# kennege/pvnet

Hardware: AMD Instinct MI355X
Metric: images/sec (480x640, 9 kp) vote->keypoint (higher is better)
Workload: dtype f32; 1 GPU; stream of LINEMOD-cat-sized batch-1 frames (configs[1]'s voting layer): ransac_voting_layer_v3 (hn=512, thr=0.99) from seg_pred/vertex_pred; one step = one hipGraph replay voting 1024 frames per GPU, 8 in flight on separate streams; images sharded round-robin over ranks, one gather of all keypoints at the end; global_batch=1024, keypoints=9, round_hyp_num=512, foreground_px=29861, parallelism=dp1 (images sharded round-robin, RCCL all_gather of keypoints), images_in_flight=8, stream_images=169984

## Files before the change

### pvnet_amd/csrc/pvvote.hip

```cpp
#include "pv_stages.h"

#define PV_VERSION "pvvote 0.2 (gfx950)"

#ifdef PVV_TRACE
#define PVV_TRACE_ON(a) ((a).trace != nullptr)
#else
#define PVV_TRACE_ON(a) false
#endif

#ifdef PVV_PROFILE
namespace pvv __attribute__((visibility("hidden"))) {
int g_abl = 0;
}
#endif

namespace {

using namespace pvv;

struct alignas(16) F4 { float x, y, z, w; };
struct alignas(8) F2 { float x, y; };

struct VoteArgs {
    const float4 *pex;
// ... 541 lines not shown
#endif

__global__ __launch_bounds__(256) void k_hyp_gen(VoteArgs a) {
    const int64_t per = (int64_t)a.nh * a.vn;
    const int64_t gid = (int64_t)blockIdx.x * 256 + threadIdx.x;
    if (gid >= per * a.b) return;
    const int b = (int)(gid / per);
    const int r = (int)(gid - b * per);
    const int h = r / a.vn, v = r - h * a.vn;
    const int n = tn_at(a, b);
    if (n > 0) a.hypv_out[((int64_t)b * a.vn + v) * a.nh + h] = item_hyp<true, true>(a, b, v, h, true, n, true);
}

typedef _Float16 h4f __attribute__((ext_vector_type(4)));
typedef float f32x16 __attribute__((ext_vector_type(16)));

constexpr int kMB = 16;
constexpr int kMChunk = PVM_CHUNK;
constexpr int kMSlots = (kMChunk + 255) / 256;
constexpr int kMBatch = kMChunk / kMB;
static_assert(kMChunk % kMB == 0 && kMBatch <= 32 && kMChunk <= 512, "hit masks: 2 x 64 bits; queue: 9-bit pixel");
constexpr int kMSet = 4;
constexpr float kMHypMax = 8.0e6f;
constexpr float kMRMax = 30000.f;
constexpr int kMQueue = PVM_QUEUE;
constexpr int kMBandK = 1;

template <bool PREPPED>
struct MSlab {
    uint4 rows[kMBatch][2 * kMB];
    ExactSlab<PREPPED, kMChunk> x;
};

__device__ __forceinline__ uint32_t pack_h2(_Float16 lo, _Float16 hi) {
    return (uint32_t)__builtin_bit_cast(uint16_t, lo) | ((uint32_t)__builtin_bit_cast(uint16_t, hi) << 16);
}

__device__ __forceinline__ uint4 form_row(float ax, float ay, float b) {
    const _Float16 axh = (_Float16)ax, axl = (_Float16)(ax - (float)axh);
    const _Float16 ayh = (_Float16)ay, ayl = (_Float16)(ay - (float)ayh);
    const float nb = -b;
    const _Float16 bh = (_Float16)nb, bl = (_Float16)(nb - (float)bh);
    return make_uint4(pack_h2(axh, axh), pack_h2(axl, ayh), pack_h2(ayh, ayl), pack_h2(bh, bl));
}

template <bool PREPPED>
__global__ __launch_bounds__(256) __attribute__((amdgpu_waves_per_eu(PVM_WPE, PVM_WPE))) void k_vote_mfma(VoteArgs a) {
    const int lane = lane_id();
    const int wid = (int)__builtin_amdgcn_readfirstlane(threadIdx.x / kWave);
    const int col = lane & 31, half = lane >> 5;
    const int unit = (int)blockIdx.x;
    const uint32_t nunits = gridDim.x;
    const uint64_t t_start = __builtin_amdgcn_s_memrealtime();
    __builtin_amdgcn_s_setprio(3);
    __shared__ MSlab<PREPPED> slab[2];
    __shared__ QuarterBoxes qb_all[2];
    __shared__ float2 hyp_all[4 * kGroup];
    __shared__ uint32_t bq_all[4][kMQueue];
    __shared__ int32_t corr_all[4][kGroup];
    float2 *hlds = hyp_all + wid * kGroup;
    uint32_t *bq = bq_all[wid];
    int32_t *corr = corr_all[wid];
    const int ggn = a.hgn / 4;
    uint32_t total = 0;
    for (int b = 0; b < a.b; ++b) total += (uint32_t)(a.vn * ggn) * (uint32_t)tn_at(a, b);
    uint32_t lo, hi;
    if (a.rw[0] > 0 && nunits % (a.rw[3] > 0 ? 4 : 3) == 0) {
        round_share(total, nunits, (uint32_t)unit, a.rw, &lo, &hi);
    } else {
        even_share(total, nunits, (uint32_t)unit, &lo, &hi);
    }
    int buf = 0, nfix = 0, nseg = 0, nslow = 0, nxo = 0, nqd = 0;
    uint64_t tloop = 0, t_total = 0, t_hyp = 0;
    uint64_t c_stage = 0, c_hot = 0, c_fix = 0, c_seg = 0, c_mark = 0;
    uint64_t c_band = 0, c_flush = 0, c_xo = 0;
    auto cyc = [&]() -> uint64_t { return PVV_TRACE_ON(a) ? __builtin_amdgcn_s_memtime() : 0; };
    if (PVV_TRACE_ON(a)) t_total = __builtin_amdgcn_s_memrealtime();
    const float tau = a.tau;
    constexpr float kBig = 3.0e38f;
    int b = 0;
    uint32_t base = 0;
    while (lo < hi && b < a.b) {
        const int n = tn_at(a, b);
        const uint32_t span = (uint32_t)(a.vn * ggn) * (uint32_t)n;
        if (lo >= base + span) { base += span; ++b; continue; }
        const uint32_t r0 = lo - base;
        const int g = (int)(r0 / (uint32_t)n);
        const int ts = uniform((int)(r0 - (uint32_t)g * n));
        const int te = uniform((int)min((uint32_t)n, ts + (hi - lo)));
        const int v = uniform(g / ggn), gg = g - (g / ggn) * ggn;
        const int hg = uniform(gg * 4 + wid);
        c_mark = cyc();
        F4 L[kMSlots];
        auto load_px = [&](int s0, int np) {
#pragma unroll
            for (int k = 0; k < kMSlots; ++k) {
                const int t = k * 256 + wid * kWave + lane;
                L[k] = F4{0.f, 0.f, 0.f, 0.f};
                if (t < np) L[k] = pixel_exact<PREPPED>(a, b, v, s0 + t);
            }
        };
        load_px(ts, min(kMChunk, te - ts));
        uint32_t hfm = 0, hxm = 0;
#pragma unroll
        for (int i = 0; i < 2; ++i) {
            const int h = hg * kGroup + i * kWave + lane;
            const bool hl = h < a.nh;
            const float2 hv = a.hyp ? item_hyp<false, PREPPED>(a, b, v, h, hl, n, false)
                                    : item_hyp<PREPPED, PREPPED>(a, b, v, h, hl, n, PREPPED && ts == 0);
            hlds[i * kWave + lane] = hv;
        }
        __builtin_amdgcn_wave_barrier();
#pragma unroll
        for (int j = 0; j < kMSet; ++j) {
            const int h = hg * kGroup + j * 32 + col;
            const float2 hv = hlds[j * 32 + col];
            const bool fin = isfinite(hv.x) && isfinite(hv.y);
            const bool xo = h < a.nh && fin &&
                            (hyp_exact_only(hv.x, hv.y) || !(fabsf(hv.x) < kMHypMax && fabsf(hv.y) < kMHypMax));
            hxm |= xo ? 1u << j : 0u;
            hfm |= (h < a.nh && fin && !xo) ? 1u << j : 0u;
        }
        int cnt[kMSet] = {0, 0, 0, 0};
        corr[lane] = 0;
        corr[64 + lane] = 0;
        if (PVV_TRACE_ON(a) && t_hyp == 0) t_hyp = __builtin_amdgcn_s_memrealtime();
        for (int s0 = ts; s0 < te; s0 += kMChunk) {
            {
                const uint64_t t = cyc();
                if (s0 == ts) c_seg += t - c_mark; else c_fix += t - c_mark;
                c_mark = t;
            }
            const int np = uniform(min(kMChunk, te - s0));
            MSlab<PREPPED> &S = slab[buf];
            QuarterBoxes &QB = qb_all[buf];
            buf ^= 1;
            const int t = wid * kWave + lane;
            bool exo_p = false;
            float xl = kBig, xh = -kBig;
            float4 q[kMSlots];
            float yq[kMSlots];
#pragma unroll
            for (int k = 0; k < kMSlots; ++k) {
                const int tt = k * 256 + t;
                q[k] = make_float4(__builtin_nanf(""), 0.f, 0.f, 0.f);
                yq[k] = 0.f;
                if (tt < np) {
                    const F4 e = L[k];
                    bool ex = false;
                    if (PREPPED) q[k] = prep_compacted(e, &ex);
                    else { q[k] = prep_pixel(e.x, e.y, e.z, e.w); ex = pixel_exotic(e.z, e.w); }
                    exo_p |= ex;
                    S.x.put(tt, e);
                    xl = fminf(xl, e.x); xh = fmaxf(xh, e.x); yq[k] = q[k].y;
                }
            }
            if (wid * kWave < np) {
                const float mn = wave_min(xl), mx = wave_max(xh);
                float yn, yx;
                if (PREPPED) {
                    yn = bcast(yq[0], 0);
                    const bool s1 = kMSlots > 1 && 256 + wid * kWave < np;
                    yx = s1 ? bcast(yq[kMSlots - 1], min(kWave - 1, np - 1 - 256 - wid * kWave))
                            : bcast(yq[0], min(kWave - 1, np - 1 - wid * kWave));
                } else {
                    float mnq = kBig, mxq = -kBig;
#pragma unroll
                    for (int k = 0; k < kMSlots; ++k)
                        if (k * 256 + t < np) { mnq = fminf(mnq, yq[k]); mxq = fmaxf(mxq, yq[k]); }
                    yn = wave_min(mnq);
                    yx = wave_max(mxq);
                }
                const uint32_t ex = __builtin_amdgcn_ballot_w64(exo_p) != 0;
                if (lane == 0) { QB.box[wid] = make_float4(mn, mx, yn, yx); QB.exo[wid] = ex; }
            } else if (lane == 0) {
                QB.box[wid] = make_float4(kBig, -kBig, kBig, -kBig);
                QB.exo[wid] = 0;
            }
            auto put_rows = [&](float ox, float oy, bool slow) {
#pragma unroll
                for (int k = 0; k < kMSlots; ++k) {
                    const int tt = k * 256 + t;
                    if (tt >= kMChunk) break;
                    uint4 rx = make_uint4(0u, 0u, pack_h2((_Float16)0.f, (_Float16)0.f),
                                          pack_h2((_Float16)(-60000.f), (_Float16)0.f));
                    uint4 ry = make_uint4(0u, 0u, 0u, 0u);
                    if (q[k].x == q[k].x && !slow) {
                        const float cx = q[k].x - ox, cy = q[k].y - oy;
                        const float axX = tau * q[k].z, ayX = tau * q[k].w;
                        rx = form_row(axX, ayX, fmaf(axX, cx, ayX * cy));
                        ry = form_row(-q[k].w, q[k].z, fmaf(-q[k].w, cx, q[k].z * cy));
                    }
                    S.rows[tt >> 4][2 * (tt & 15)] = rx;
                    S.rows[tt >> 4][2 * (tt & 15) + 1] = ry;
                }
            };
            if (s0 + kMChunk < te) load_px(s0 + kMChunk, min(kMChunk, te - s0 - kMChunk));
            __syncthreads();
            float cxl = kBig, cxh = -kBig, cyl = kBig, cyh = -kBig;
            uint32_t exq = 0;
#pragma unroll
            for (int k = 0; k < 4; ++k) {
                const float4 Q = QB.box[k];
                cxl = fminf(cxl, Q.x); cxh = fmaxf(cxh, Q.y);
                cyl = fminf(cyl, Q.z); cyh = fmaxf(cyh, Q.w);
                exq |= QB.exo[k];
            }
            float ox = floorf(0.5f * cxl + 0.5f * cxh), oy = floorf(0.5f * cyl + 0.5f * cyh);
            if (!(fabsf(ox) <= 1.6e7f && fabsf(oy) <= 1.6e7f)) { ox = 0.f; oy = 0.f; }
            const float axr = fmaxf(cxh - ox, ox - cxl), ayr = fmaxf(cyh - oy, oy - cyl);
            const float R = __builtin_amdgcn_sqrtf(fmaf(axr, axr, ayr * ayr)) * 1.00001f;
            bool slow = !a.fast || exq != 0 || !(R * fmaxf(tau, 1.f) <= kMRMax);
            slow = __builtin_amdgcn_readfirstlane(slow);
            nslow += slow ? 1 : 0;
            put_rows(ox, oy, slow);
            __syncthreads();
            if (!slow) {
                auto hscale = [&](int j, float &hx, float &hy, float &s, float &Bv) {
                    const bool fj = (hfm >> j) & 1u;
                    const float2 hv = hlds[j * 32 + col];
                    hx = hv.x - ox;
                    hy = hv.y - oy;
                    const float mag = fmaxf(fabsf(hx), fabsf(hy));
                    const int e = __builtin_amdgcn_frexp_expf(mag);
                    const int k = fj ? max(0, e - 14) : 0;
                    s = __builtin_ldexpf(1.f, -k);
                    Bv = (__builtin_amdgcn_sqrtf(fmaf(hx, hx, hy * hy)) * 1.00001f + R) * 1.00001f + 1.f;
                };
                h4f bf[kMSet];
                float gb[kMSet];
#pragma unroll
                for (int j = 0; j < kMSet; ++j) {
                    const bool fj = (hfm >> j) & 1u;
                    float hx, hy, s, Bv;
                    hscale(j, hx, hy, s, Bv);
                    const float hxs = hx * s, hys = hy * s;
                    const _Float16 xh_ = (_Float16)hxs, xl_ = (_Float16)(hxs - (float)xh_);
                    const _Float16 yh_ = (_Float16)hys, yl_ = (_Float16)(hys - (float)yh_);
                    const _Float16 sh = (_Float16)s;
                    h4f f = half ? h4f{yl_, yh_, sh, sh} : h4f{xh_, xl_, xh_, yh_};
                    if (!fj) f = h4f{(_Float16)0.f, (_Float16)0.f, (_Float16)0.f, (_Float16)0.f};
                    bf[j] = f;
                    gb[j] = fj ? (a.gzf + a.gzr) * Bv * s * 1.00001f : -1.f;
                }
                uint32_t neg[kMSet] = {0u, 0u, 0u, 0u};
                uint64_t hm0 = 0, hm1 = 0;
                const int nb = (np + kMB - 1) / kMB;
                const uint2 *arow = (const uint2 *)&S.rows[0][0];
                auto afrag = [&](int p) -> h4f {
                    const uint2 w = arow[(p * kMB * 2 + col) * 2 + half];
                    return __builtin_bit_cast(h4f, w);
                };
                auto zvals = [&](const f32x16 &c, float z[8]) {
#pragma unroll
                    for (int q = 0; q < 8; ++q) z[q] = c[2 * q] - fabsf(c[2 * q + 1]);
                };
                auto proc = [&](const f32x16 &c, uint32_t &ng) -> float {
                    float z[8];
                    zvals(c, z);
#pragma unroll
                    for (int q = 0; q < 8; q += 4) {
                        const uint32_t p01 = __builtin_amdgcn_perm(__float_as_uint(z[q + 1]), __float_as_uint(z[q]), 0x0c0c0b09u);
                        const uint32_t p23 = __builtin_amdgcn_perm(__float_as_uint(z[q + 3]), __float_as_uint(z[q + 2]), 0x0b090c0cu);
                        ng = __builtin_amdgcn_sad_u8(p01, p23, ng);
                    }
                    float mb = __builtin_elementwise_minimum(__builtin_elementwise_minimum(fabsf(z[0]), fabsf(z[1])), fabsf(z[2]));
                    mb = __builtin_elementwise_minimum(__builtin_elementwise_minimum(mb, fabsf(z[3])), fabsf(z[4]));
                    mb = __builtin_elementwise_minimum(__builtin_elementwise_minimum(mb, fabsf(z[5])), fabsf(z[6]));
                    return __builtin_elementwise_minimum(mb, fabsf(z[7]));
                };
                const f32x16 zero = {};
                if (PVV_TRACE_ON(a) && tloop == 0) tloop = __builtin_amdgcn_s_memrealtime();
                { const uint64_t t = cyc(); c_stage += t - c_mark; c_mark = t; }
                h4f A = afrag(0);
                f32x16 c0 = __builtin_amdgcn_mfma_f32_32x32x8f16(A, bf[0], zero, 0, 0, 0);
#pragma unroll 1
                for (int p = 0; p < nb; ++p) {
                    const h4f An = afrag(min(p + 1, kMBatch - 1));
                    const f32x16 c1 = __builtin_amdgcn_mfma_f32_32x32x8f16(A, bf[1], zero, 0, 0, 0);
                    const float m0 = proc(c0, neg[0]);
                    const f32x16 c2 = __builtin_amdgcn_mfma_f32_32x32x8f16(A, bf[2], zero, 0, 0, 0);
                    const float m1 = proc(c1, neg[1]);
                    const f32x16 c3 = __builtin_amdgcn_mfma_f32_32x32x8f16(A, bf[3], zero, 0, 0, 0);
                    const float m2 = proc(c2, neg[2]);
                    c0 = __builtin_amdgcn_mfma_f32_32x32x8f16(An, bf[0], zero, 0, 0, 0);
                    const float m3 = proc(c3, neg[3]);
                    const uint32_t hb = (__builtin_amdgcn_ballot_w64(m0 <= gb[0]) != 0 ? 1u : 0u) |
                                        (__builtin_amdgcn_ballot_w64(m1 <= gb[1]) != 0 ? 2u : 0u) |
                                        (__builtin_amdgcn_ballot_w64(m2 <= gb[2]) != 0 ? 4u : 0u) |
                                        (__builtin_amdgcn_ballot_w64(m3 <= gb[3]) != 0 ? 8u : 0u);
                    const uint64_t hbs = (uint64_t)hb << ((p & 15) * kMSet);
                    if (p < 16) hm0 |= hbs; else hm1 |= hbs;
                    A = An;
                }
#pragma unroll
                for (int j = 0; j < kMSet; ++j) cnt[j] += ((hfm >> j) & 1u) ? 8 * nb - (int)(neg[j] / 255u) : 0;
                { const uint64_t t = cyc(); c_hot += t - c_mark; c_mark = t; }
#ifdef PVV_PROFILE
                if (a.rw[3] == 7777) hm0 = hm1 = 0;
#endif
                const float kx = a.gzr / tau * 1.0001f, ky = a.gzr * 1.0001f;
                int nq = 0;
                auto flush = [&]() {
                    for (int k0 = 0; k0 < nq; k0 += kWave) {
                        if (k0 + lane < nq) {
                            const uint32_t en = bq[k0 + lane];
                            const int pix = (int)(en & 0x1ffu), jj = (int)((en >> 9) & 3u), cl = (int)((en >> 11) & 31u);
                            const int f = (int)(en >> 16) & 1;
                            const F4 e = S.x.get(pix);
                            const float2 hj = hlds[jj * 32 + cl];
                            const int r = exact_vote(e.z, e.w, e.x, e.y, hj.x, hj.y, a.thr) ? 1 : 0;
                            if (r != f) atomicAdd(&corr[jj * 32 + cl], r - f);
                        }
                    }
                    nq = 0;
                };
                const float inv1k = 1.0002f / (1.f - ky * 1.0001f);
                float Gs[kMSet];
                const float gq = a.gzf / (a.gzf + a.gzr) * 1.0011f * inv1k;
#pragma unroll
                for (int j = 0; j < kMSet; ++j) Gs[j] = gb[j] * gq;
                const float Kb = (kx + ky) * inv1k;
                auto band_test = [&](const f32x16 &c, int p, int j) {
                    const bool fj = (hfm >> j) & 1u;
                    const float G = j == 0 ? Gs[0] : j == 1 ? Gs[1] : j == 2 ? Gs[2] : Gs[3];
                    float zs[8], ts[8];
#pragma unroll
                    for (int q = 0; q < 8; ++q) {
                        const float X = c[2 * q], Y = c[2 * q + 1];
                        zs[q] = X - fabsf(Y);
                        ts[q] = fmaf(-Kb, fabsf(X), fabsf(zs[q]));
                    }
                    float mt = __builtin_elementwise_minimum(__builtin_elementwise_minimum(ts[0], ts[1]), ts[2]);
                    mt = __builtin_elementwise_minimum(__builtin_elementwise_minimum(mt, ts[3]), ts[4]);
                    mt = __builtin_elementwise_minimum(__builtin_elementwise_minimum(mt, ts[5]), ts[6]);
                    mt = __builtin_elementwise_minimum(mt, ts[7]);
#ifdef PVV_PROFILE
                    if (a.rw[3] == 7778) mt = 3.0e38f;
#endif
                    if (__builtin_amdgcn_ballot_w64(fj && mt <= G)) {
#pragma unroll
                        for (int q = 0; q < 8; ++q) {
                            const int pix = p * kMB + (q & 1) + 4 * (q >> 1) + 2 * half;
                            const bool u = fj && pix < np && ts[q] <= G;
                            const uint64_t m = __builtin_amdgcn_ballot_w64(u);
                            if (m) {
                                if (nq > kMQueue - kWave) flush();
                                const int at = nq + (int)__builtin_amdgcn_mbcnt_hi((uint32_t)(m >> 32), __builtin_amdgcn_mbcnt_lo((uint32_t)m, 0u));
                                if (u) bq[at] = (uint32_t)pix | ((uint32_t)j << 9) | ((uint32_t)col << 11) | ((signbit(zs[q]) ? 0u : 1u) << 16);
                                nq += __popcll(m);
                                nqd += __popcll(m);
                            }
                        }
                    }
                };
                static_assert(kMSet == 4, "band selects");
                auto bsel = [&](int j) -> h4f { return j == 0 ? bf[0] : j == 1 ? bf[1] : j == 2 ? bf[2] : bf[3]; };
                while (hm0 | hm1) {
                    int pk[kMBandK], jk[kMBandK], nk = 0;
#pragma unroll
                    for (int k = 0; k < kMBandK; ++k) {
                        pk[k] = 0; jk[k] = 0;
                        if (hm0 | hm1) {
                            int bit;
                            if (hm0) { bit = __builtin_ctzll(hm0); hm0 &= hm0 - 1; }
                            else { bit = 64 + __builtin_ctzll(hm1); hm1 &= hm1 - 1; }
                            pk[k] = bit / kMSet; jk[k] = bit % kMSet;
                            nk = k + 1;
                        }
                    }
                    nfix += nk;
                    h4f ak[kMBandK];
#pragma unroll
                    for (int k = 0; k < kMBandK; ++k) ak[k] = afrag(pk[k]);
                    f32x16 ck[kMBandK];
#pragma unroll
                    for (int k = 0; k < kMBandK; ++k)
                        ck[k] = __builtin_amdgcn_mfma_f32_32x32x8f16(ak[k], bsel(jk[k]), zero, 0, 0, 0);
#pragma unroll
                    for (int k = 0; k < kMBandK; ++k)
                        if (k < nk) band_test(ck[k], pk[k], jk[k]);
                }
                { const uint64_t t = cyc(); c_band += t - c_mark; c_fix += t - c_mark; c_mark = t; }
                flush();
                __builtin_amdgcn_wave_barrier();
                { const uint64_t t = cyc(); c_flush += t - c_mark; c_fix += t - c_mark; c_mark = t; }
#pragma unroll
                for (int j = 0; j < kMSet; ++j) {
                    uint64_t mm = __builtin_amdgcn_ballot_w64(((hxm >> j) & 1u) && half == 0);
                    nxo += __popcll(mm);
                    while (mm) {
                        const int l = __builtin_ctzll(mm);
                        mm &= mm - 1;
                        const float2 hx2 = hlds[j * 32 + l];
                        int c = 0;
#pragma unroll
                        for (int k = 0; k < (kMChunk + kWave - 1) / kWave; ++k) {
                            const int jj = k * kWave + lane;
                            bool e = false;
                            if (jj < np) {
                                const F4 x = S.x.get(jj);
                                e = exact_vote(x.z, x.w, x.x, x.y, hx2.x, hx2.y, a.thr);
                            }
                            c += __popcll(__builtin_amdgcn_ballot_w64(e));
                        }
                        if (lane == l) cnt[j] += c;
                    }
                }
                { const uint64_t t = cyc(); c_xo += t - c_mark; c_fix += t - c_mark; c_mark = t; }
            } else {
#pragma unroll 1
                for (int jj = half; jj < np; jj += 2) {
                    const F4 e = S.x.get(jj);
#pragma unroll
                    for (int j = 0; j < kMSet; ++j)
                        if ((hfm | hxm) >> j & 1u) {
                            const float2 hv = hlds[j * 32 + col];
                            cnt[j] += exact_vote(e.z, e.w, e.x, e.y, hv.x, hv.y, a.thr);
                        }
                }
            }
        }
        __builtin_amdgcn_wave_barrier();
#pragma unroll
        for (int j = 0; j < kMSet; ++j) cnt[j] += half == 0 ? corr[j * 32 + col] : 0;
        int32_t *cp = a.counts + (int64_t)b * a.cnt_bs + (int64_t)v * a.cnt_v;
#pragma unroll
        for (int j = 0; j < kMSet; ++j) {
            const auto sw = __builtin_amdgcn_permlane32_swap(cnt[j], cnt[j], false, false);
            const int tot = (int)(sw[0] + sw[1]);
            const int h = hg * kGroup + j * 32 + col;
            if (half == 0 && h < a.nh && tot) atomicAdd(&cp[(int64_t)h * a.cnt_h], tot);
        }
        lo += te - ts;
        ++nseg;
        { const uint64_t t = cyc(); c_fix += t - c_mark; c_mark = t; }
    }
    if (PVV_TRACE_ON(a) && lane == 0) {
        const int wave = (int)(blockIdx.x * 4 + wid);
        uint64_t *q = a.trace + 65536 + wave * 8;
        q[0] = c_seg; q[1] = c_stage; q[2] = c_hot; q[3] = c_fix;
        q[4] = c_band; q[5] = c_flush; q[6] = c_xo; q[7] = (uint64_t)nqd;
    }
    if (PVV_TRACE_ON(a) && lane == 0) {
        const int wave = (int)(blockIdx.x * 4 + wid);
        uint32_t hw, xcc;
        asm volatile("s_getreg_b32 %0, hwreg(HW_REG_HW_ID)" : "=s"(hw));
        asm volatile("s_getreg_b32 %0, hwreg(HW_REG_XCC_ID)" : "=s"(xcc));
        a.trace[wave * 8] = t_start;
        a.trace[wave * 8 + 1] = __builtin_amdgcn_s_memrealtime();
        a.trace[wave * 8 + 2] = ((uint64_t)xcc << 32) | hw;
        a.trace[wave * 8 + 3] = ((uint64_t)nseg << 32) | (uint32_t)nfix;
        a.trace[wave * 8 + 4] = tloop;
        a.trace[wave * 8 + 5] = ((uint64_t)nslow << 32) | (uint32_t)nxo;
        a.trace[wave * 8 + 6] = t_total;
        a.trace[wave * 8 + 7] = t_hyp;
    }
}


__global__ __launch_bounds__(256) void k_generate_api(const float *direct, const float *coords, const int32_t *idxs,
                                                      float *hypo, int tn, int vn, int hn) {
    int hv = blockIdx.x * 256 + threadIdx.x;
    if (hv >= hn * vn) return;
    int hi = hv / vn, vi = hv - hi * vn;
    int t0 = idxs[hi * vn * 2 + vi * 2], t1 = idxs[hi * vn * 2 + vi * 2 + 1];
    float x = 0.f, y = 0.f, ox, oy;
    if (t0 >= 0 && t0 < tn && t1 >= 0 && t1 < tn &&
        exact_intersect(direct[t0 * vn * 2 + vi * 2], direct[t0 * vn * 2 + vi * 2 + 1], coords[t0 * 2],
                        coords[t0 * 2 + 1], direct[t1 * vn * 2 + vi * 2], direct[t1 * vn * 2 + vi * 2 + 1],
                        coords[t1 * 2], coords[t1 * 2 + 1], &ox, &oy)) {
        x = ox; y = oy;
    }
    hypo[hi * vn * 2 + vi * 2] = x;
    hypo[hi * vn * 2 + vi * 2 + 1] = y;
}

constexpr int kBytePix = 8;
constexpr int kByteWin = kWave * kBytePix;
constexpr int kByteHB = PVV_BYTE_HB;
static_assert(kByteHB <= 64 && kByteHB % 16 == 0, "row masks are 64-bit; quarter blocks take 16 rows");
constexpr uint32_t kQueuePerWave = 128;

#ifdef PVVOTE_TRACE_U1
__device__ uint64_t *g_btrace;
#endif

struct ByteArgs {
    const float *direct;
    const float *coords;
    const float *hypo;
    uint8_t *out;
    int tn, vn, hn, nwin, nhg, fast;
    float thr, tau, gzf, gzr;
    int dbg;
    int xcd;
    int bal_t, bal_nt, bal_tnx, bal_ttx;
};

__device__ __forceinline__ float4 api_pixel(const float2 c, const float2 d) {
    const float n1 = sqrtf(d.x * d.x + d.y * d.y);
    const bool ok = !below_1e6(n1) && n1 == n1 && isfinite(c.x) && isfinite(c.y);
    const float rs = __builtin_amdgcn_rsqf(fmaf(d.x, d.x, d.y * d.y));
    float4 q = make_float4(0.f, 0.f, c.x, c.y);
    if (ok)
        q = (n1 <= kN1Max) ? make_float4(d.x * rs, d.y * rs, c.x, c.y)
                           : make_float4(__builtin_nanf(""), 0.f, c.x, c.y);
    return q;
}
__device__ __forceinline__ float2 api_coords(const ByteArgs &a, int t) {
    return *(const float2 *)(a.coords + (int64_t)t * 2);
}
__device__ __forceinline__ float2 api_direct(const ByteArgs &a, int t, int v) {
    return *(const float2 *)(a.direct + ((int64_t)t * a.vn + v) * 2);
}

__device__ __forceinline__ void prio_by_remaining(uint32_t remaining, uint32_t total) {
    const uint64_t r3 = (uint64_t)remaining * 3, w1 = (uint64_t)total + 1;
    if (r3 >= 2 * w1) __builtin_amdgcn_s_setprio(2);
    else if (r3 >= w1) __builtin_amdgcn_s_setprio(1);
    else __builtin_amdgcn_s_setprio(0);
}

struct WinInfo {
    float ox, oy, bxl, bxh, byl, byh, Rw;
    int slow;
};

template <int MODE>
__device__ __forceinline__ void vote_bytes_seg(const ByteArgs &a, F4 *recs, uint8_t *band8, int v, int w, int h0,
                                               int nh, uint32_t rem_after, uint32_t wave_total, uint16_t *wq,
                                               uint32_t &qn, uint64_t *tsetup, const float4 *stage, float2 hq,
                                               const float4 *raw, const float2 *hraw, const WinInfo *win) {
    const uint32_t qcap = a.dbg == 4 ? 1u : kQueuePerWave;
    const int lane = lane_id();
    const float ntau = -a.tau;
    const int tb = kByteWin * w + kBytePix * lane;
    const int64_t rstep = (int64_t)a.vn * a.tn;
    int64_t obase = ((int64_t)h0 * a.vn + v) * a.tn + (int64_t)kByteWin * w;
    obase = (int64_t)((uint64_t)(uint32_t)__builtin_amdgcn_readfirstlane((int)(obase >> 32)) << 32 |
                      (uint32_t)__builtin_amdgcn_readfirstlane((int)obase));
    const uint32_t loff = kBytePix * lane;

    uint32_t vmask = 0;
    float fu[kBytePix], fv[kBytePix], fk1[kBytePix], fk2[kBytePix];
    float ox = 0.f, oy = 0.f, Rw = 0.f, bxl = 0.f, bxh = 0.f, byl = 0.f, byh = 0.f;
    bool slow;
    if (stage) {
#pragma unroll
        for (int j = 0; j < kBytePix; ++j) {
            fu[j] = fv[j] = fk2[j] = 0.f;
            fk1[j] = -1.0e30f;
            if (tb + j < a.tn) {
                const float4 q = stage[j * kWave + lane];
                fu[j] = q.x; fv[j] = q.y; fk1[j] = q.z; fk2[j] = q.w;
                vmask |= 1u << j;
            }
        }
        slow = __builtin_amdgcn_readfirstlane(!a.fast || win->slow);
        ox = win->ox; oy = win->oy; Rw = win->Rw;
        bxl = win->bxl; bxh = win->bxh; byl = win->byl; byh = win->byh;
        __syncthreads();
    } else {
        uint32_t okmask = 0;
        bool exo = false;
        float2 c[kBytePix], d[kBytePix];
#pragma unroll
        for (int j = 0; j < kBytePix; ++j) {
            const int t = tb + j;
            c[j] = d[j] = make_float2(0.f, 0.f);
            if (t < a.tn) {
                c[j] = api_coords(a, t);
                d[j] = api_direct(a, t, v);
                vmask |= 1u << j;
            }
        }
#pragma unroll
        for (int j = 0; j < kBytePix; ++j) {
            const float4 q = api_pixel(c[j], d[j]);
            const bool in = vmask >> j & 1;
            fu[j] = in ? q.x : 0.f; fv[j] = in ? q.y : 0.f; fk1[j] = in ? q.z : 0.f; fk2[j] = in ? q.w : 0.f;
        }
#pragma unroll
        for (int j = 0; j < kBytePix; ++j) {
            exo |= fu[j] != fu[j];
            if (fu[j] != 0.f || fv[j] != 0.f) okmask |= 1u << j;
        }
        slow = __builtin_amdgcn_readfirstlane(!a.fast || __builtin_amdgcn_ballot_w64(exo) != 0);
        const uint64_t anyok = __builtin_amdgcn_ballot_w64(okmask != 0);
        if (anyok) {
            const int l0 = __builtin_ctzll(anyok);
            const int j0 = __builtin_ctz(__builtin_amdgcn_readlane(okmask, l0));
            float fx = fk1[0], fy = fk2[0];
#pragma unroll
            for (int j = 1; j < kBytePix; ++j)
                if (j == j0) { fx = fk1[j]; fy = fk2[j]; }
            ox = floorf(bcast(fx, l0));
            oy = floorf(bcast(fy, l0));
            float xl = 3.0e38f, xh = -3.0e38f, yl = 3.0e38f, yh = -3.0e38f;
#pragma unroll
            for (int j = 0; j < kBytePix; ++j)
                if (okmask >> j & 1) {
                    xl = fminf(xl, fk1[j] - ox); xh = fmaxf(xh, fk1[j] - ox);
                    yl = fminf(yl, fk2[j] - oy); yh = fmaxf(yh, fk2[j] - oy);
                }
            bxl = wave_min(xl); bxh = wave_max(xh);
            byl = wave_min(yl); byh = wave_max(yh);
            const float ax = fmaxf(-bxl, bxh), ay = fmaxf(-byl, byh);
            Rw = __builtin_amdgcn_sqrtf(fmaf(ax, ax, ay * ay)) * 1.00001f;
        }
#pragma unroll
        for (int j = 0; j < kBytePix; ++j) {
            const bool ok = okmask >> j & 1;
            const float ux = fu[j], uy = fv[j];
            const float cx = fk1[j] - ox, cy = fk2[j] - oy;
            fu[j] = ok ? ux : 0.f;
            fv[j] = ok ? uy : 0.f;
            fk1[j] = ok ? -fmaf(ux, cx, uy * cy) : -1.0e30f;
            fk2[j] = ok ? -fmaf(ux, cy, -(uy * cx)) : 0.f;
        }
    }
    uint64_t flagged;
    {
        F4 rec{0.f, 0.f, __builtin_inff(), 1.f};
        if (lane < nh) {
            const bool xo = !(isfinite(hq.x) && isfinite(hq.y)) || hyp_exact_only(hq.x, hq.y);
            if (!xo && !slow) {
                const float hx = hq.x - ox, hy = hq.y - oy;
                const float B = (__builtin_amdgcn_sqrtf(fmaf(hx, hx, hy * hy)) + Rw) * 1.00001f + 1e-30f;
                const float dx = fmaxf(fabsf(hx - bxl), fabsf(hx - bxh));
                const float dy = fmaxf(fabsf(hy - byl), fabsf(hy - byh));
                const float D = fmaf(__builtin_amdgcn_sqrtf(fmaf(dx, dx, dy * dy)), 1.00001f, B * 1e-6f);
                rec = F4{hx, hy, fmaf(a.gzr, D, a.gzf * B) * 1.00001f, 0.f};
            }
        }
        flagged = __builtin_amdgcn_ballot_w64(lane < nh && rec.w != 0.f);
        __builtin_amdgcn_wave_barrier();
        if (lane < kByteHB) recs[lane] = rec;
        __builtin_amdgcn_wave_barrier();
    }

    typedef uint64_t u64a1 __attribute__((aligned(1)));
    auto store = [&](uint8_t *p, uint32_t lo, uint32_t hi, auto partial) {
        if (!decltype(partial)::value || vmask == 0xffu) {
            const uint64_t x = (uint64_t)hi << 32 | lo;
            if (MODE == PV_VOTE_DENSE) {
                *(u64a1 *)p = x;
            } else {
                const uint64_t old = *(const u64a1 *)p;
                *(u64a1 *)p = (old & ~(x * 0xffu)) | x;
            }
        } else if (vmask) {
            typedef uint32_t u32a1 __attribute__((aligned(1)));
            typedef uint16_t u16a1 __attribute__((aligned(1)));
            const int n = __builtin_popcount(vmask);
            uint64_t x = (uint64_t)hi << 32 | lo;
            int o = 0;
            if (n & 4) {
                const uint32_t y = (uint32_t)x;
                if (MODE == PV_VOTE_DENSE) *(u32a1 *)(p + o) = y;
                else *(u32a1 *)(p + o) = (*(const u32a1 *)(p + o) & ~(y * 0xffu)) | y;
                x >>= 32;
                o += 4;
            }
            if (n & 2) {
                const uint16_t y = (uint16_t)x;
                if (MODE == PV_VOTE_DENSE) *(u16a1 *)(p + o) = y;
                else *(u16a1 *)(p + o) = (uint16_t)((*(const u16a1 *)(p + o) & ~(y * 0xffu)) | y);
                x >>= 16;
                o += 2;
            }
            if (n & 1) {
                const uint8_t y = (uint8_t)x;
                if (MODE == PV_VOTE_DENSE) p[o] = y;
                else if (y) p[o] = 1;
            }
        }
    };
    constexpr uint32_t kSgn01 = 0x0c0c0b09u;
    constexpr uint32_t kSgn23 = 0x0b090c0cu;
    auto pack4 = [&](float z0, float z1, float z2, float z3) {
        const uint32_t p01 = __builtin_amdgcn_perm(__float_as_uint(z1), __float_as_uint(z0), kSgn01);
        const uint32_t p23 = __builtin_amdgcn_perm(__float_as_uint(z3), __float_as_uint(z2), kSgn23);
        return (p01 | p23) & 0x01010101u;
    };
    auto zrow = [&](const F4 &rec, float nz[kBytePix]) {
        float m = 3.0e38f;
#pragma unroll
        for (int j = 0; j < kBytePix; ++j) {
// ... 902 lines not shown
```

Baseline: 57170 images/sec.

## Compact band-test hits into per-lane bitmasks and enqueue them with one ballot

Restructures the band re-check loop so each flagged MFMA tile yields a per-lane 8-bit hit mask and a sign mask, built with inline v_cmp/v_addc and alignbit, instead of eight separate ballots and mbcnt prefix computations. Lanes with hits are then packed into the fix-up queue through a readlane prefix walk. If the queue overflows, the tile is held over for the next pass after a flush. The per-set enable is folded into the threshold by setting it to -inf, which removes the per-lane fj tests. The loop now handles one MFMA at a time (kMBandK==1) and uses a switch for B-fragment selection, trading MFMA batching for less ballot and branch overhead.

```diff
diff --git a/pvnet_amd/csrc/pvvote.hip b/pvnet_amd/csrc/pvvote.hip
--- a/pvnet_amd/csrc/pvvote.hip
+++ b/pvnet_amd/csrc/pvvote.hip
@@ -867,6 +867,7 @@
                 const float kx = a.gzr / tau * 1.0001f, ky = a.gzr * 1.0001f;
                 int nq = 0;
                 auto flush = [&]() {
+                    nqd += nq;
                     for (int k0 = 0; k0 < nq; k0 += kWave) {
                         if (k0 + lane < nq) {
                             const uint32_t en = bq[k0 + lane];
@@ -884,11 +885,11 @@
                 float Gs[kMSet];
                 const float gq = a.gzf / (a.gzf + a.gzr) * 1.0011f * inv1k;
 #pragma unroll
-                for (int j = 0; j < kMSet; ++j) Gs[j] = gb[j] * gq;
+                for (int j = 0; j < kMSet; ++j) Gs[j] = ((hfm >> j) & 1u) ? gb[j] * gq : -__builtin_inff();
                 const float Kb = (kx + ky) * inv1k;
-                auto band_test = [&](const f32x16 &c, int p, int j) {
-                    const bool fj = (hfm >> j) & 1u;
-                    const float G = j == 0 ? Gs[0] : j == 1 ? Gs[1] : j == 2 ? Gs[2] : Gs[3];
+                uint32_t cm = 0, sm = 0;
+                auto band_test = [&](const f32x16 &c, int p, float G) {
+                    cm = 0;
                     float zs[8], ts[8];
 #pragma unroll
                     for (int q = 0; q < 8; ++q) {
@@ -903,53 +904,71 @@
 #ifdef PVV_PROFILE
                     if (a.rw[3] == 7778) mt = 3.0e38f;
 #endif
-                    if (__builtin_amdgcn_ballot_w64(fj && mt <= G)) {
-#pragma unroll
-                        for (int q = 0; q < 8; ++q) {
-                            const int pix = p * kMB + (q & 1) + 4 * (q >> 1) + 2 * half;
-                            const bool u = fj && pix < np && ts[q] <= G;
-                            const uint64_t m = __builtin_amdgcn_ballot_w64(u);
-                            if (m) {
-                                if (nq > kMQueue - kWave) flush();
-                                const int at = nq + (int)__builtin_amdgcn_mbcnt_hi((uint32_t)(m >> 32), __builtin_amdgcn_mbcnt_lo((uint32_t)m, 0u));
-                                if (u) bq[at] = (uint32_t)pix | ((uint32_t)j << 9) | ((uint32_t)col << 11) | ((signbit(zs[q]) ? 0u : 1u) << 16);
-                                nq += __popcll(m);
-                                nqd += __popcll(m);
-                            }
+                    if (__builtin_amdgcn_ballot_w64(mt <= G)) {
+                        uint32_t um = 0;
+                        sm = 0;
+#pragma unroll
+                        for (int q = 7; q >= 0; --q) {
+                            asm("v_cmp_le_f32_e32 vcc, %1, %2\n\tv_addc_co_u32_e32 %0, vcc, %0, %0, vcc"
+                                : "+v"(um) : "v"(ts[q]), "v"(G) : "vcc");
+                            sm = __builtin_amdgcn_alignbit(sm, __float_as_uint(zs[q]), 31);
+                        }
+                        if (p * kMB + kMB > np) {
+                            uint32_t vm = 0;
+#pragma unroll
+                            for (int q = 0; q < 8; ++q)
+                                vm |= (p * kMB + (q & 1) + 4 * (q >> 1) + 2 * half < np) ? 1u << q : 0u;
+                            um &= vm;
+                        }
+                        cm = um;
+                    }
+                };
+                static_assert(kMBandK == 1, "the re-check loop is written for one flagged MFMA at a time");
+                static_assert(kMSet == 4, "band sets");
+                int pc = 0, jc = 0;
+                bool kept = false;
+                for (;;) {
+                    if (!kept && (hm0 | hm1)) {
+                        int bit;
+                        if (hm0) { bit = __builtin_ctzll(hm0); hm0 &= hm0 - 1; }
+                        else { bit = 64 + __builtin_ctzll(hm1); hm1 &= hm1 - 1; }
+                        pc = bit / kMSet; jc = bit % kMSet;
+                        ++nfix;
+                        const h4f ak = afrag(pc);
+                        switch (jc) {
+                        case 0: band_test(__builtin_amdgcn_mfma_f32_32x32x8f16(ak, bf[0], zero, 0, 0, 0), pc, Gs[0]); break;
+                        case 1: band_test(__builtin_amdgcn_mfma_f32_32x32x8f16(ak, bf[1], zero, 0, 0, 0), pc, Gs[1]); break;
+                        case 2: band_test(__builtin_amdgcn_mfma_f32_32x32x8f16(ak, bf[2], zero, 0, 0, 0), pc, Gs[2]); break;
+                        default: band_test(__builtin_amdgcn_mfma_f32_32x32x8f16(ak, bf[3], zero, 0, 0, 0), pc, Gs[3]); break;
                         }
                     }
-                };
-                static_assert(kMSet == 4, "band selects");
-                auto bsel = [&](int j) -> h4f { return j == 0 ? bf[0] : j == 1 ? bf[1] : j == 2 ? bf[2] : bf[3]; };
-                while (hm0 | hm1) {
-                    int pk[kMBandK], jk[kMBandK], nk = 0;
-#pragma unroll
-                    for (int k = 0; k < kMBandK; ++k) {
-                        pk[k] = 0; jk[k] = 0;
-                        if (hm0 | hm1) {
-                            int bit;
-                            if (hm0) { bit = __builtin_ctzll(hm0); hm0 &= hm0 - 1; }
-                            else { bit = 64 + __builtin_ctzll(hm1); hm1 &= hm1 - 1; }
-                            pk[k] = bit / kMSet; jk[k] = bit % kMSet;
-                            nk = k + 1;
+                    const uint64_t lm = __builtin_amdgcn_ballot_w64(cm != 0u);
+                    if (lm) {
+                        const int cnt = __popc(cm);
+                        int at = 0, tot = nq;
+                        for (uint64_t w = lm; w; w &= w - 1) {
+                            const int l = __builtin_ctzll(w);
+                            at = lane == l ? tot : at;
+                            tot += __builtin_amdgcn_readlane(cnt, l);
                         }
+                        for (uint32_t m = cm; m && at < kMQueue; m &= m - 1, ++at) {
+                            const int q = __builtin_ctz(m);
+                            const int pix = pc * kMB + (q & 1) + 4 * (q >> 1) + 2 * half;
+                            bq[at] = (uint32_t)pix | ((uint32_t)jc << 9) | ((uint32_t)col << 11) | ((~(sm >> q) & 1u) << 16);
+                            cm &= cm - 1;
+                        }
+                        kept = tot > kMQueue;
+                        nq = min(tot, kMQueue);
                     }
-                    nfix += nk;
-                    h4f ak[kMBandK];
-#pragma unroll
-                    for (int k = 0; k < kMBandK; ++k) ak[k] = afrag(pk[k]);
-                    f32x16 ck[kMBandK];
-#pragma unroll
-                    for (int k = 0; k < kMBandK; ++k)
-                        ck[k] = __builtin_amdgcn_mfma_f32_32x32x8f16(ak[k], bsel(jk[k]), zero, 0, 0, 0);
-#pragma unroll
-                    for (int k = 0; k < kMBandK; ++k)
-                        if (k < nk) band_test(ck[k], pk[k], jk[k]);
-                }
-                { const uint64_t t = cyc(); c_band += t - c_mark; c_fix += t - c_mark; c_mark = t; }
-                flush();
-                __builtin_amdgcn_wave_barrier();
-                { const uint64_t t = cyc(); c_flush += t - c_mark; c_fix += t - c_mark; c_mark = t; }
+                    const bool last = !kept && !(hm0 | hm1);
+                    if (kept || last) {
+                        { const uint64_t t = cyc(); c_band += t - c_mark; c_fix += t - c_mark; c_mark = t; }
+                        if (nq) flush();
+                        __builtin_amdgcn_wave_barrier();
+                        { const uint64_t t = cyc(); c_flush += t - c_mark; c_fix += t - c_mark; c_mark = t; }
+                    }
+                    if (last) break;
+                }
 #pragma unroll
                 for (int j = 0; j < kMSet; ++j) {
                     uint64_t mm = __builtin_amdgcn_ballot_w64(((hxm >> j) & 1u) && half == 0);
```

Result: no change. 57680 images/sec (median of 6 runs) (+0.9%).
